# AIM-Harvard/pyradiomics

Hardware: NVIDIA H100
Metric: voxels/s full-texture voxel-based (higher is better)
Workload: dtype f64

## Files before the change

pyradiomics_b200/csrc/small_fast.cuh:

```cuda
#pragma once
#include "glcm_fast.cuh"

namespace rb {

struct SmallFastTables {
  double log2t[32];
  double inv2[256];
  double invsq[32];
  double rcp[64];
};

inline void small_fast_build_tables(SmallFastTables& T) {
  T.log2t[0] = 0; T.invsq[0] = 0; T.inv2[0] = 0; T.rcp[0] = 0;
  for (int c = 1; c < 32; c++) { T.log2t[c] = log2((double)c); T.invsq[c] = 1.0 / ((double)c * c); }
  for (int g = 1; g < 256; g++) T.inv2[g] = 1.0 / ((double)g * g);
  for (int c = 1; c < 64; c++) T.rcp[c] = 1.0 / (double)c;
}

RB_HD constexpr uint32_t nb26(int v) {
  uint32_t m = 0;
  const int z = v / 9, y = (v / 3) % 3, x = v % 3;
  for (int dz = -1; dz <= 1; dz++) for (int dy = -1; dy <= 1; dy++) for (int dx = -1; dx <= 1; dx++) {
    if (!dz && !dy && !dx) continue;
    const int z2 = z + dz, y2 = y + dy, x2 = x + dx;
    if (z2 < 0 || z2 > 2 || y2 < 0 || y2 > 2 || x2 < 0 || x2 > 2) continue;
    m |= 1u << (z2 * 9 + y2 * 3 + x2);
  }
  return m;
}
template <int V> struct NB26 { static constexpr uint32_t value = nb26(V); };

template <int V, int END> struct ForPos {
  template <typename F> static RB_HD void go(F& f) { f.template at<V>(); ForPos<V + 1, END>::go(f); }
};
template <int END> struct ForPos<END, END> { template <typename F> static RB_HD void go(F&) {} };

struct GldmPass1 {
  const int* wl; const uint32_t* cl; int* dep; uint32_t M;
  template <int V> RB_HD void at() { dep[V] = wl[V] ? (int)RB_POPC(cl[V] & NB26<V>::value) : -1 - V; }
};

RB_HD void gldm_fast_voxel(const int* wl, int alpha, const SmallFastTables& T, double* out) {
  uint32_t eq[27];
  RB_EQMASKS_27(wl, eq);
  uint32_t cl[27];
  if (alpha == 0) {
#pragma unroll
    for (int v = 0; v < 27; v++) cl[v] = eq[v];
  } else {
#pragma unroll
    for (int v = 0; v < 27; v++) cl[v] = 0;
#pragma unroll
    for (int p = 0; p < 27; p++)
#pragma unroll
      for (int q = p + 1; q < 27; q++) {
        const int d = wl[p] - wl[q];
        if (wl[p] && wl[q] && d <= alpha && -d <= alpha) { cl[p] |= 1u << q; cl[q] |= 1u << p; }
      }
  }
  int dep[27];
  GldmPass1 p1{wl, cl, dep, 0};
  ForPos<0, 27>::go(p1);
  uint32_t dq[27];
  RB_EQMASKS_27_KEY(dep, dq);
  int Nz = 0, Sj = 0, Sj2 = 0, B = 0, C = 0, X4 = 0, gl = 0, dn = 0;
  double Sinv = 0, A = 0, X1 = 0, X2 = 0, X3 = 0, lg = 0;
#pragma unroll
  for (int v = 0; v < 27; v++) {
    if (wl[v]) {
      const int g = wl[v], g2 = g * g, j = dep[v] + 1, j2 = j * j;
      const double ig = T.inv2[g], ij = T.invsq[j];
      Nz++; Sj += j; Sj2 += j2; B += g2; C += g; X4 += g2 * j2;
      Sinv += ij; A += ig; X1 += ig * ij; X2 += g2 * ij; X3 += j2 * ig;
      gl += RB_POPC(eq[v]); dn += RB_POPC(dq[v]);
      lg += T.log2t[RB_POPC(eq[v] & dq[v])];
    }
  }
  const double inv = 1.0 / Nz, inv2 = inv * inv;
  out[0] = T.log2t[Nz] - lg * inv;
  out[1] = dn * inv;
  out[2] = dn * inv2;
  out[3] = (double)(Nz * Sj2 - Sj * Sj) * inv2;
  out[4] = gl * inv;
  out[5] = (double)(Nz * B - C * C) * inv2;
  out[6] = B * inv;
  out[7] = Sj2 * inv;
  out[8] = X4 * inv;
  out[9] = X3 * inv;
  out[10] = A * inv;
  out[11] = Sinv * inv;
  out[12] = X2 * inv;
  out[13] = X1 * inv;
}

constexpr int NGTDM_L = 34034;

RB_HD constexpr int ngtdm_full_cnt(int v) {
  return (v % 3 == 1 ? 3 : 2) * ((v / 3) % 3 == 1 ? 3 : 2) * (v / 9 == 1 ? 3 : 2) - 1;
}

RB_HD double ngtdm_i2d(int d) {
#ifdef __CUDA_ARCH__
  return __hiloint2double(0x43300000, d) - 4503599627370496.0;
#else
  return (double)d;
#endif
}

RB_HD double ngtdm_complexity_pairs(const int* pk, const double* ns, int st, int nl, const SmallFastTables& T) {
  double c0 = 0, c1 = 0;
  for (int a = 0; a + 1 < nl; a++) {
    const int pa = pk[a * st], na = pa >> 8, ia = pa & 255;
    const double sa = ns[a * st];
    int b = a + 1;
    for (; b + 1 < nl; b += 2) {
      const int p0 = pk[b * st], p1 = pk[(b + 1) * st];
      const int x0 = ia - (p0 & 255), x1 = ia - (p1 & 255);
      c0 += ngtdm_i2d(x0 < 0 ? -x0 : x0) * ((sa + ns[b * st]) * T.rcp[na + (p0 >> 8)]);
      c1 += ngtdm_i2d(x1 < 0 ? -x1 : x1) * ((sa + ns[(b + 1) * st]) * T.rcp[na + (p1 >> 8)]);
    }
    if (b < nl) {
      const int p0 = pk[b * st], x0 = ia - (p0 & 255);
      c0 += ngtdm_i2d(x0 < 0 ? -x0 : x0) * ((sa + ns[b * st]) * T.rcp[na + (p0 >> 8)]);
    }
  }
  return c0 + c1;
}

struct NgtdmGeneralDiff {
  const int* wl; const uint32_t* eq; uint32_t M; const SmallFastTables* T; double* scr_ns; int st; double ssum;
  template <int V> RB_HD void at() {
    if (!wl[V]) return;
    constexpr uint32_t nb = NB26<V>::value;
    int sum = 0;
#pragma unroll
    for (int u = 0; u < 27; u++) if (nb >> u & 1u) sum += wl[u];
    const int cnt = RB_POPC(M & nb), x = cnt * wl[V] - sum;
    const double d = ngtdm_i2d(x < 0 ? -x : x) * T->rcp[cnt];
    ssum += d;
    const int r = RB_CTZ(eq[V]);
    const double prev = r == V ? 0.0 : scr_ns[r * st];
    scr_ns[r * st] = prev + d;
  }
};

template <bool FULL>
RB_HD void ngtdm_fast_body(const int* wl, const SmallFastTables& T, double* out, int* scr_pk, double* scr_ns, int st) {
  int B = 0, C = 0;
#pragma unroll
  for (int v = 0; v < 27; v++) { B += wl[v] * wl[v]; C += wl[v]; }
  uint32_t eq[27];
  RB_EQMASKS_27(wl, eq);
  int Nvp = 27, SE = 0;
  double ssum = 0;
  if (FULL) {
    int bx[27], by[27], bz[27];
#pragma unroll
    for (int r = 0; r < 27; r += 3) {
      bx[r] = wl[r] + wl[r + 1]; bx[r + 1] = bx[r] + wl[r + 2]; bx[r + 2] = wl[r + 1] + wl[r + 2];
    }
#pragma unroll
    for (int r = 0; r < 27; r += 9)
#pragma unroll
      for (int x = 0; x < 3; x++) {
        const int* b = bx + r + x;
        by[r + x] = b[0] + b[3]; by[r + 3 + x] = by[r + x] + b[6]; by[r + 6 + x] = b[3] + b[6];
      }
#pragma unroll
    for (int yx = 0; yx < 9; yx++) {
      bz[yx] = by[yx] + by[9 + yx]; bz[9 + yx] = bz[yx] + by[18 + yx]; bz[18 + yx] = by[9 + yx] + by[18 + yx];
    }
#pragma unroll
    for (int v = 0; v < 27; v++) {
      const int cnt = ngtdm_full_cnt(v);
      const int x = (cnt + 1) * wl[v] - bz[v];
      const int e = (x < 0 ? -x : x) * (NGTDM_L / cnt);
      SE += e;
      const int r = RB_CTZ(eq[v]);
      const int prev = r == v ? 0 : scr_pk[r * st];
      scr_pk[r * st] = prev + e;
    }
  } else {
    uint32_t M = 0;
#pragma unroll
    for (int v = 0; v < 27; v++) if (wl[v]) M |= 1u << v;
    Nvp = RB_POPC(M);
    NgtdmGeneralDiff p1{wl, eq, M, &T, scr_ns, st, 0.0};
    ForPos<0, 27>::go(p1);
    ssum = p1.ssum;
  }
  int nl = 0, SL = 0, SL2 = 0;
  double pw = 0;
  int X[27];
#pragma unroll
  for (int v = 0; v < 27; v++) {
    const bool rep = eq[v] && (eq[v] & ((1u << v) - 1)) == 0;
    const int n = RB_POPC(eq[v]), g = wl[v];
    const double ns = FULL ? ngtdm_i2d(n) * ngtdm_i2d(scr_pk[v * st]) : ngtdm_i2d(n) * scr_ns[v * st];
    scr_pk[nl * st] = n << 8 | g;
    scr_ns[nl * st] = ns;
    X[v] = rep ? g * n : 0;
    if (rep) { nl++; SL += g; SL2 += g * g; pw += ns; }
  }
  RB_NGTDM_SORT27(X);
  int bd = 0;
#pragma unroll
  for (int k = 0; k < 27; k++) bd += (2 * k - 53 + nl) * X[k];
  const double cpx = ngtdm_complexity_pairs(scr_pk, scr_ns, st, nl, T);
  const double u = FULL ? (double)NGTDM_L : 1.0, N = (double)Nvp;
  const double sdiff = FULL ? (double)SE : ssum;
  out[N_Coarseness] = pw != 0 ? N * u / pw : 1e6;
  const double div = (double)nl * (nl - 1);
  out[N_Contrast] = div != 0 ? 2.0 * (double)(Nvp * B - C * C) * sdiff / (N * N * N * u * div) : 0.0;
  out[N_Busyness] = bd != 0 ? pw / (2.0 * u * (double)bd) : 0.0;
  out[N_Complexity] = 2.0 * cpx / (N * u);
  out[N_Strength] = sdiff != 0 ? 2.0 * u * (double)(nl * B - 2 * C * SL + Nvp * SL2) / (N * sdiff) : 0.0;
}

RB_HD bool ngtdm_window_full(const int* wl) {
  bool full = true;
#pragma unroll
  for (int v = 0; v < 27; v++) full &= wl[v] != 0;
  return full;
}

RB_HD void ngtdm_fast_voxel(const int* wl, const SmallFastTables& T, double* out) {
  int pk[27] = {0};
  double ns[27] = {0};
  if (ngtdm_window_full(wl)) ngtdm_fast_body<true>(wl, T, out, pk, ns, 1);
  else ngtdm_fast_body<false>(wl, T, out, pk, ns, 1);
}

RB_HD uint32_t dilate26(uint32_t m) {
  constexpr uint32_t X0 = 0x1249249u, X2 = 0x4924924u;
  constexpr uint32_t Y0 = 0x01C0E07u, Y2 = 0x70381C0u;
  m |= ((m & ~X2) << 1) | ((m & ~X0) >> 1);
  m |= ((m & ~Y2) << 3) | ((m & ~Y0) >> 3);
  m |= (m << 9) | (m >> 9);
  return m & 0x7FFFFFFu;
}

struct GlszmAcc {
  int Nz, Sg, Sg2, Ss2, X4, gln;
  double A, Sinv, X1, X2, X3, lg;
  unsigned long long h0, h1, h2;
};

RB_HD void glszm_fast_voxel(const int* wl, const SmallFastTables& T, double* out) {
  uint32_t eq[27];
  RB_EQMASKS_27(wl, eq);
  uint32_t M = 0;
  uint32_t cls[13];
  int clg[13];
  int nl = 0, S_n = 0, S_g = 0, S_g2 = 0;
  double S_ig = 0;
#pragma unroll
  for (int v = 0; v < 27; v++) {
    if (wl[v]) M |= 1u << v;
    if (eq[v] && (eq[v] & ((1u << v) - 1)) == 0) {
      if (eq[v] == (1u << v)) { S_n++; S_g += wl[v]; S_g2 += wl[v] * wl[v]; S_ig += T.inv2[wl[v]]; }
      else { cls[nl] = eq[v]; clg[nl] = wl[v]; nl++; }
    }
  }
  GlszmAcc a;
  a.Nz = S_n; a.Sg = S_g; a.Sg2 = S_g2; a.Ss2 = S_n; a.X4 = S_g2; a.gln = S_n;
  a.A = S_ig; a.Sinv = (double)S_n; a.X1 = S_ig; a.X2 = (double)S_g2; a.X3 = S_ig; a.lg = 0;
  a.h0 = (unsigned long long)S_n; a.h1 = a.h2 = 0;
  for (int k = 0; k < nl; k++) {
    const int g = clg[k], g2 = g * g;
    uint32_t m = cls[k];
    const double ig = T.inv2[g];
    int zs[8];
    int zc = 0;
    while (m && zc < 8) {
      uint32_t comp = m & (0u - m);
      for (;;) {
        const uint32_t nx = dilate26(comp) & m;
        if (nx == comp) break;
        comp = nx;
      }
      m &= ~comp;
      const int sz = RB_POPC(comp), s2 = sz * sz;
      zs[zc++] = sz;
      const double is = T.invsq[sz];
      a.Nz++; a.Sg += g; a.Sg2 += g2; a.Ss2 += s2; a.X4 += g2 * s2;
      a.A += ig; a.Sinv += is; a.X1 += ig * is; a.X2 += g2 * is; a.X3 += s2 * ig;
      if (sz <= 12) a.h0 += 1ull << (5 * (sz - 1));
      else if (sz <= 24) a.h1 += 1ull << (5 * (sz - 13));
      else a.h2 += 1ull << (5 * (sz - 25));
    }
    a.gln += zc * zc;
    for (int k = 0; k < zc; k++) {
      int c = 0;
      for (int l = 0; l < zc; l++) c += zs[l] == zs[k];
      a.lg += T.log2t[c];
    }
  }
  int szn = 0;
#pragma unroll
  for (int k = 0; k < 12; k++) {
    const int c0 = (int)(a.h0 >> (5 * k)) & 31, c1 = (int)(a.h1 >> (5 * k)) & 31;
    szn += c0 * c0 + c1 * c1;
  }
#pragma unroll
  for (int k = 0; k < 3; k++) { const int c2 = (int)(a.h2 >> (5 * k)) & 31; szn += c2 * c2; }
  const int Np = RB_POPC(M), Nz = a.Nz;
  const double inv = 1.0 / Nz, inv2 = inv * inv;
  out[S_GLN] = a.gln * inv; out[S_GLNN] = a.gln * inv2;
  out[S_GLV] = (double)(Nz * a.Sg2 - a.Sg * a.Sg) * inv2;
  out[S_HGLE] = a.Sg2 * inv; out[S_LargeE] = a.Ss2 * inv; out[S_LargeHGLE] = a.X4 * inv; out[S_LargeLGLE] = a.X3 * inv;
  out[S_LGLE] = a.A * inv; out[S_SizeNU] = szn * inv; out[S_SizeNUN] = szn * inv2; out[S_SmallE] = a.Sinv * inv;
  out[S_SmallHGLE] = a.X2 * inv; out[S_SmallLGLE] = a.X1 * inv;
  out[S_Entropy] = T.log2t[Nz] - a.lg * inv;
  out[S_Percentage] = (double)Nz / Np;
  out[S_SizeVar] = (double)(Nz * a.Ss2 - Np * Np) * inv2;
}

}
```

pyradiomics_b200/csrc/voxel_fast.cu:

```cuda
#include <map>
#include <mutex>

#include "common.cuh"
#define RB_GLCM_BLOCK_SYNC 1
#include "glcm_fast.cuh"
#include "glcm_kernels.cuh"
#include "glrlm_fast.cuh"
#include "small_fast.cuh"
#include "host_common.hpp"

namespace rb {

bool glcm_fast_applicable(int cls, int level_bytes, const VoxParams& P) {
  return cls == C_GLCM && level_bytes == 1 && P.rz == 1 && P.ry == 1 && P.rx == 1 && P.na == 13 && P.symmetric &&
         !P.weighted && P.Ng <= 255;
}

struct GlcmQueue { GlcmTask* q = nullptr; double* res = nullptr; unsigned* count = nullptr; size_t cap = 0; };
static std::mutex g_queue_mu;
static std::map<std::pair<int, cudaStream_t>, GlcmQueue> g_queue_cache;
int glcm_release_queues() {
  int dev = 0;
  if (cudaGetDevice(&dev) != cudaSuccess) return RB_ERR_CUDA;
  cudaDeviceSynchronize();
  std::lock_guard<std::mutex> lk(g_queue_mu);
  for (auto it = g_queue_cache.begin(); it != g_queue_cache.end();) {
    if (it->first.first == dev) {
      cudaFree(it->second.q); cudaFree(it->second.res); cudaFree(it->second.count);
      it = g_queue_cache.erase(it);
    } else ++it;
  }
  return RB_OK;
}
static GlcmQueue* glcm_queue(cudaStream_t st, size_t need) {
  std::mutex& mu = g_queue_mu;
  auto& cache = g_queue_cache;
  int dev = 0;
  if (cudaGetDevice(&dev) != cudaSuccess) return nullptr;
  std::lock_guard<std::mutex> lk(mu);
  GlcmQueue& Q = cache[{dev, st}];
  if (!Q.count && cudaMalloc(&Q.count, sizeof(unsigned)) != cudaSuccess) return nullptr;
  if (Q.cap < need) {
    if (Q.q) { cudaStreamSynchronize(st); cudaFree(Q.q); cudaFree(Q.res); Q.q = nullptr; Q.res = nullptr; Q.cap = 0; }
    if (cudaMalloc(&Q.q, need * sizeof(GlcmTask)) != cudaSuccess) return nullptr;
    if (cudaMalloc(&Q.res, need * sizeof(double)) != cudaSuccess) { cudaFree(Q.q); Q.q = nullptr; return nullptr; }
    Q.cap = need;
  }
  return &Q;
}

int glcm_fast_launch(const void* lev, const uint8_t* centers, const VoxParams& P, double* out, long long fstride,
                     int z0, int z1, int out_z0, cudaStream_t st) {
  const GlcmFastTables* T = device_table<GlcmFastTables>([&](GlcmFastTables& h) { glcm_fast_build_tables(h, P.Ng); }, P.Ng);
  if (!T) return fail(RB_ERR_CUDA, "could not build the GLCM table block on the device");
  const long long plane = (long long)P.Y * P.X;
  if ((long long)(z1 - z0) * plane <= 0) return RB_OK;
  if (P.sy != P.X || P.sz != plane) return fail(RB_ERR_ARG, "GLCM fast path expects a contiguous level volume");
  const int sms = sm_count();
  const long long max_entries = 48ll << 20;
  int zchunk = (int)(max_entries / (plane * GF_NA));
  if (zchunk < 1) zchunk = 1;
  if (zchunk > z1 - z0) zchunk = z1 - z0;
  GlcmQueue* Q = glcm_queue(st, (size_t)zchunk * plane * GF_NA);
  if (!Q) return fail(RB_ERR_NOMEM, "could not allocate the GLCM eigen-task queue");
  constexpr int NT = 512;
  const int smem = glcm_phaseA_smem_bytes(NT);
  RB_CUDA(set_max_dynamic_smem(glcm_fast_kernel<1, NT>, smem));
  RB_CUDA(set_max_dynamic_smem(glcm_fast_solve_kernel<2>, GF_LZ_SMEM_BYTES));
  const uint8_t* l8 = (const uint8_t*)lev;
  for (int za = z0; za < z1; za += zchunk) {
    const int zb = za + zchunk < z1 ? za + zchunk : z1;
    RB_CUDA(cudaMemsetAsync(Q->count, 0, sizeof(unsigned), st));
    int grid = 0;
    RB_CUDA(resident_grid(glcm_fast_kernel<1, NT>, NT, smem, (long long)(zb - za) * plane, grid));
    glcm_fast_kernel<1, NT><<<grid, NT, smem, st>>>(l8, centers, P, T, out, fstride, za, zb, out_z0, Q->q, Q->count);
    RB_LAUNCH_CHECK();
    glcm_fast_solve_kernel<0><<<sms * 8, 128, 0, st>>>(l8, P, T, Q->q, Q->count, Q->res, 0);
    for (int g = 10; g <= 12; g += 2) glcm_fast_solve_kernel<1><<<sms * 8, 128, 0, st>>>(l8, P, T, Q->q, Q->count, Q->res, g);
    for (int g = 18; g >= 14; g -= 2)
      glcm_fast_solve_kernel<2><<<sms * 2, 128, GF_LZ_SMEM_BYTES, st>>>(l8, P, T, Q->q, Q->count, Q->res, g);
    RB_LAUNCH_CHECK();
    glcm_fast_finish_kernel<<<sms * 8, 256, 0, st>>>(P, Q->q, Q->count, Q->res, out + (long long)G_MCC * fstride, out_z0);
    RB_LAUNCH_CHECK();
  }
  return RB_OK;
}

__global__ void __launch_bounds__(128)
glrlm_fast_kernel(const uint8_t* __restrict__ lev, const uint8_t* __restrict__ centers,
                  const __grid_constant__ VoxParams P, const GlrlmFastTables* __restrict__ Tg,
                  double* __restrict__ out, long long fstride, int z0, int z1, int out_z0) {
  __shared__ GlrlmFastTables T;
  copy_tables_to_shared(T, Tg);
  __syncthreads();
  const long long plane = (long long)P.Y * P.X;
  const long long total = (long long)(z1 - z0) * plane;
  for (long long t = (long long)blockIdx.x * blockDim.x + threadIdx.x; t < total; t += (long long)gridDim.x * blockDim.x) {
    const ChunkVoxel v = chunk_voxel(P, plane, z0, out_z0, t);
    if (!chunk_center(lev, centers, plane, v)) {
#pragma unroll
      for (int k = 0; k < GLRLM_NF; k++) out[k * fstride + v.oi] = P.init_value;
      continue;
    }
    int wl[27];
    load_window27(lev, P, v.z, v.y, v.x, v.vi, true, wl, 1);
    double f[GLRLM_NF];
    glrlm_fast_voxel(wl, T, f);
#pragma unroll
    for (int k = 0; k < GLRLM_NF; k++) out[k * fstride + v.oi] = f[k];
  }
}

bool glrlm_fast_applicable(int cls, int level_bytes, const VoxParams& P) {
  return cls == C_GLRLM && level_bytes == 1 && P.rz == 1 && P.ry == 1 && P.rx == 1 && P.na == 13 && !P.weighted && P.Ng <= 255;
}

int glrlm_fast_launch(const void* lev, const uint8_t* centers, const VoxParams& P, double* out, long long fstride,
                      int z0, int z1, int out_z0, cudaStream_t st) {
  const GlrlmFastTables* T = device_table<GlrlmFastTables>(glrlm_fast_build_tables);
  if (!T) return fail(RB_ERR_CUDA, "could not build the GLRLM table block on the device");
  const long long total = (long long)(z1 - z0) * P.Y * P.X;
  if (total <= 0) return RB_OK;
  glrlm_fast_kernel<<<grid_for(total, 128, 32), 128, 0, st>>>((const uint8_t*)lev, centers, P, T, out, fstride, z0, z1, out_z0);
  RB_LAUNCH_CHECK();
  return RB_OK;
}

template <int CLS, int NT, bool SYNC>
__global__ void __launch_bounds__(NT)
small_fast_kernel(const uint8_t* __restrict__ lev, const uint8_t* __restrict__ centers,
                  const __grid_constant__ VoxParams P, const SmallFastTables* __restrict__ Tg,
                  double* __restrict__ out, long long fstride, int z0, int z1, int out_z0) {
  __shared__ SmallFastTables T;
  copy_tables_to_shared<NT>(T, Tg);
  __syncthreads();
  constexpr int NF = CLS == C_GLSZM ? GLSZM_NF : GLDM_NF;
  const long long plane = (long long)P.Y * P.X;
  const long long total = (long long)(z1 - z0) * plane;
  const long long ntiles = (total + NT - 1) / NT;
  for (long long tile = blockIdx.x; tile < ntiles; tile += gridDim.x) {
    if (SYNC) __syncthreads();
    const long long t = tile * NT + threadIdx.x;
    const bool live = t < total;
    if (!SYNC && !live) continue;
    const ChunkVoxel v = chunk_voxel(P, plane, z0, out_z0, t, live);
    const bool is_center = live && chunk_center(lev, centers, plane, v);
    if (!SYNC && !is_center) {
#pragma unroll
      for (int k = 0; k < NF; k++) out[k * fstride + v.oi] = P.init_value;
      continue;
    }
    int wl[27];
    load_window27(lev, P, v.z, v.y, v.x, v.vi, is_center, wl, 1);
    double f[16];
    if (CLS == C_GLSZM) glszm_fast_voxel(wl, T, f);
    else gldm_fast_voxel(wl, P.alpha, T, f);
    if (!live) continue;
#pragma unroll
    for (int k = 0; k < NF; k++) out[k * fstride + v.oi] = is_center ? f[k] : P.init_value;
  }
}

constexpr int NGTDM_NT = 128;
template <int NT>
__global__ void __launch_bounds__(NT, 4)
ngtdm_fast_kernel(const uint8_t* __restrict__ lev, const uint8_t* __restrict__ centers,
                  const __grid_constant__ VoxParams P, const SmallFastTables* __restrict__ Tg,
                  double* __restrict__ out, long long fstride, int z0, int z1, int out_z0) {
  __shared__ SmallFastTables T;
  __shared__ double ng_ns[27 * NT];
  __shared__ int ng_pk[27 * NT];
  __shared__ long long defer[2 * NT];
  __shared__ unsigned ndefer;
  copy_tables_to_shared<NT>(T, Tg);
  const int tid = threadIdx.x;
  if (tid == 0) ndefer = 0;
  __syncthreads();
  const long long plane = (long long)P.Y * P.X;
  full_window_tiles<NT>((long long)(z1 - z0) * plane, defer, ndefer,
    [&](long long t, bool live, auto defer_it) {
      if (!live) return;
      const ChunkVoxel v = chunk_voxel(P, plane, z0, out_z0, t);
      const bool is_center = chunk_center(lev, centers, plane, v);
      int wl[27];
      load_window27(lev, P, v.z, v.y, v.x, v.vi, is_center, wl, 1);
      if (is_center && ngtdm_window_full(wl)) {
        double f[NGTDM_NF];
        ngtdm_fast_body<true>(wl, T, f, ng_pk + tid, ng_ns + tid, NT);
#pragma unroll
        for (int k = 0; k < NGTDM_NF; k++) out[k * fstride + v.oi] = f[k];
      } else if (is_center) {
        defer_it();
      } else {
#pragma unroll
        for (int k = 0; k < NGTDM_NF; k++) out[k * fstride + v.oi] = P.init_value;
      }
    },
    [&](auto entry, bool live) {
      if (!live) return;
      const ChunkVoxel v = chunk_voxel(P, plane, z0, out_z0, entry());
      const bool is_center = chunk_center(lev, centers, plane, v);
      int wl[27];
      load_window27(lev, P, v.z, v.y, v.x, v.vi, is_center, wl, 1);
      double f[NGTDM_NF];
      ngtdm_fast_body<false>(wl, T, f, ng_pk + tid, ng_ns + tid, NT);
#pragma unroll
      for (int k = 0; k < NGTDM_NF; k++) out[k * fstride + v.oi] = f[k];
    });
}

bool small_fast_applicable(int cls, int level_bytes, const VoxParams& P) {
  return (cls == C_GLSZM || cls == C_GLDM || cls == C_NGTDM) && level_bytes == 1 && P.rz == 1 && P.ry == 1 && P.rx == 1 &&
         P.na == 26 && P.Ng <= 255;
}

int small_fast_launch(int cls, const void* lev, const uint8_t* centers, const VoxParams& P, double* out, long long fstride,
                      int z0, int z1, int out_z0, cudaStream_t st) {
  const SmallFastTables* T = device_table<SmallFastTables>(small_fast_build_tables);
  if (!T) return fail(RB_ERR_CUDA, "could not build the table block on the device");
  const long long total = (long long)(z1 - z0) * P.Y * P.X;
  if (total <= 0) return RB_OK;
  const uint8_t* l8 = (const uint8_t*)lev;
  if (cls == C_NGTDM) {
    int grid = 0;
    RB_CUDA(resident_grid(ngtdm_fast_kernel<NGTDM_NT>, NGTDM_NT, 0, total, grid));
    ngtdm_fast_kernel<NGTDM_NT><<<grid, NGTDM_NT, 0, st>>>(l8, centers, P, T, out, fstride, z0, z1, out_z0);
  } else if (cls == C_GLSZM) {
    small_fast_kernel<C_GLSZM, 128, false><<<grid_for(total, 128, 32), 128, 0, st>>>(l8, centers, P, T, out, fstride, z0, z1, out_z0);
  } else {
    small_fast_kernel<C_GLDM, 256, true><<<grid_for(total, 256, 16), 256, 0, st>>>(l8, centers, P, T, out, fstride, z0, z1, out_z0);
  }
  RB_LAUNCH_CHECK();
  return RB_OK;
}

}
```

Before: 263.9 million.

## Split GLSZM/GLDM voxel kernels into full-window fast path with deferred partial windows

Templates the GLSZM and GLDM per-voxel bodies on whether the 3x3x3 window is fully inside the mask, so the common case skips the zero checks and mask bookkeeping. Partial windows are deferred and handled in a second pass, reusing the NGTDM tiling scheme with a resident grid. GLDM computes its dependence histogram and joint entropy via packed counters and a combined key instead of a second equality-mask pass. GLSZM computes entropy incrementally with a delta-log table and keeps cluster scratch in shared memory, which adds shared memory use and relies on load_window27 returning a fullness flag.

```diff
diff --git a/pyradiomics_b200/csrc/small_fast.cuh b/pyradiomics_b200/csrc/small_fast.cuh
--- a/pyradiomics_b200/csrc/small_fast.cuh
+++ b/pyradiomics_b200/csrc/small_fast.cuh
@@ -8,6 +8,7 @@
   double inv2[256];
   double invsq[32];
   double rcp[64];
+  double dclog2[32];
 };
 
 inline void small_fast_build_tables(SmallFastTables& T) {
@@ -15,6 +16,7 @@
   for (int c = 1; c < 32; c++) { T.log2t[c] = log2((double)c); T.invsq[c] = 1.0 / ((double)c * c); }
   for (int g = 1; g < 256; g++) T.inv2[g] = 1.0 / ((double)g * g);
   for (int c = 1; c < 64; c++) T.rcp[c] = 1.0 / (double)c;
+  for (int c = 0; c < 32; c++) T.dclog2[c] = (c + 1) * log2((double)(c + 1)) - (c ? c * log2((double)c) : 0.0);
 }
 
 RB_HD constexpr uint32_t nb26(int v) {
@@ -36,13 +38,18 @@
 template <int END> struct ForPos<END, END> { template <typename F> static RB_HD void go(F&) {} };
 
 struct GldmPass1 {
-  const int* wl; const uint32_t* cl; int* dep; uint32_t M;
-  template <int V> RB_HD void at() { dep[V] = wl[V] ? (int)RB_POPC(cl[V] & NB26<V>::value) : -1 - V; }
-};
-
-RB_HD void gldm_fast_voxel(const int* wl, int alpha, const SmallFastTables& T, double* out) {
+  const uint32_t* cl; int* dep;
+  template <int V> RB_HD void at() { dep[V] = (int)RB_POPC(cl[V] & NB26<V>::value); }
+};
+
+template <bool FULL>
+RB_HD void gldm_fast_body(const int* wl, int alpha, const SmallFastTables& T, double* out) {
   uint32_t eq[27];
-  RB_EQMASKS_27(wl, eq);
+  if (FULL) RB_EQMASKS_27_KEY(wl, eq);
+  else RB_EQMASKS_27(wl, eq);
+  int gl = 0;
+#pragma unroll
+  for (int v = 0; v < 27; v++) gl += RB_POPC(eq[v]);
   uint32_t cl[27];
   if (alpha == 0) {
 #pragma unroll
@@ -55,28 +62,43 @@
 #pragma unroll
       for (int q = p + 1; q < 27; q++) {
         const int d = wl[p] - wl[q];
-        if (wl[p] && wl[q] && d <= alpha && -d <= alpha) { cl[p] |= 1u << q; cl[q] |= 1u << p; }
+        if ((FULL || (wl[p] && wl[q])) && d <= alpha && -d <= alpha) { cl[p] |= 1u << q; cl[q] |= 1u << p; }
       }
   }
   int dep[27];
-  GldmPass1 p1{wl, cl, dep, 0};
+  GldmPass1 p1{cl, dep};
   ForPos<0, 27>::go(p1);
-  uint32_t dq[27];
-  RB_EQMASKS_27_KEY(dep, dq);
-  int Nz = 0, Sj = 0, Sj2 = 0, B = 0, C = 0, X4 = 0, gl = 0, dn = 0;
+  int Nz = 0, Sj = 0, Sj2 = 0, B = 0, C = 0, X4 = 0;
   double Sinv = 0, A = 0, X1 = 0, X2 = 0, X3 = 0, lg = 0;
+  unsigned long long h0 = 0, h1 = 0, h2 = 0;
+  int key[27];
 #pragma unroll
   for (int v = 0; v < 27; v++) {
-    if (wl[v]) {
-      const int g = wl[v], g2 = g * g, j = dep[v] + 1, j2 = j * j;
+    const bool in = FULL || wl[v];
+    const int g = wl[v], g2 = g * g, j = dep[v] + 1, j2 = j * j;
+    key[v] = in ? g << 5 | dep[v] : -1 - v;
+    if (in) {
       const double ig = T.inv2[g], ij = T.invsq[j];
       Nz++; Sj += j; Sj2 += j2; B += g2; C += g; X4 += g2 * j2;
       Sinv += ij; A += ig; X1 += ig * ij; X2 += g2 * ij; X3 += j2 * ig;
-      gl += RB_POPC(eq[v]); dn += RB_POPC(dq[v]);
-      lg += T.log2t[RB_POPC(eq[v] & dq[v])];
-    }
-  }
-  const double inv = 1.0 / Nz, inv2 = inv * inv;
+      if (dep[v] < 12) h0 += 1ull << (5 * dep[v]);
+      else if (dep[v] < 24) h1 += 1ull << (5 * (dep[v] - 12));
+      else h2 += 1ull << (5 * (dep[v] - 24));
+    }
+  }
+  int dn = 0;
+#pragma unroll
+  for (int k = 0; k < 12; k++) { const int c = (int)(h0 >> (5 * k)) & 31; dn += c * c; }
+#pragma unroll
+  for (int k = 0; k < 12; k++) { const int c = (int)(h1 >> (5 * k)) & 31; dn += c * c; }
+#pragma unroll
+  for (int k = 0; k < 3; k++) { const int c = (int)(h2 >> (5 * k)) & 31; dn += c * c; }
+  uint32_t kq[27];
+  RB_EQMASKS_27_KEY(key, kq);
+#pragma unroll
+  for (int v = 0; v < 27; v++)
+    if (FULL || key[v] >= 0) lg += T.log2t[RB_POPC(kq[v])];
+  const double inv = FULL ? 1.0 / 27 : 1.0 / Nz, inv2 = inv * inv;
   out[0] = T.log2t[Nz] - lg * inv;
   out[1] = dn * inv;
   out[2] = dn * inv2;
@@ -217,7 +239,7 @@
   out[N_Strength] = sdiff != 0 ? 2.0 * u * (double)(nl * B - 2 * C * SL + Nvp * SL2) / (N * sdiff) : 0.0;
 }
 
-RB_HD bool ngtdm_window_full(const int* wl) {
+RB_HD bool window27_full(const int* wl) {
   bool full = true;
 #pragma unroll
   for (int v = 0; v < 27; v++) full &= wl[v] != 0;
@@ -227,7 +249,7 @@
 RB_HD void ngtdm_fast_voxel(const int* wl, const SmallFastTables& T, double* out) {
   int pk[27] = {0};
   double ns[27] = {0};
-  if (ngtdm_window_full(wl)) ngtdm_fast_body<true>(wl, T, out, pk, ns, 1);
+  if (window27_full(wl)) ngtdm_fast_body<true>(wl, T, out, pk, ns, 1);
   else ngtdm_fast_body<false>(wl, T, out, pk, ns, 1);
 }
 
@@ -246,20 +268,20 @@
   unsigned long long h0, h1, h2;
 };
 
-RB_HD void glszm_fast_voxel(const int* wl, const SmallFastTables& T, double* out) {
+template <bool FULL>
+RB_HD void glszm_fast_body(const int* wl, const SmallFastTables& T, double* out, unsigned long long* scr, int st) {
   uint32_t eq[27];
-  RB_EQMASKS_27(wl, eq);
+  if (FULL) RB_EQMASKS_27_KEY(wl, eq);
+  else RB_EQMASKS_27(wl, eq);
   uint32_t M = 0;
-  uint32_t cls[13];
-  int clg[13];
   int nl = 0, S_n = 0, S_g = 0, S_g2 = 0;
   double S_ig = 0;
 #pragma unroll
   for (int v = 0; v < 27; v++) {
-    if (wl[v]) M |= 1u << v;
+    if (!FULL && wl[v]) M |= 1u << v;
     if (eq[v] && (eq[v] & ((1u << v) - 1)) == 0) {
       if (eq[v] == (1u << v)) { S_n++; S_g += wl[v]; S_g2 += wl[v] * wl[v]; S_ig += T.inv2[wl[v]]; }
-      else { cls[nl] = eq[v]; clg[nl] = wl[v]; nl++; }
+      else { scr[nl * st] = eq[v] | (unsigned long long)wl[v] << 32; nl++; }
     }
   }
   GlszmAcc a;
@@ -267,12 +289,13 @@
   a.A = S_ig; a.Sinv = (double)S_n; a.X1 = S_ig; a.X2 = (double)S_g2; a.X3 = S_ig; a.lg = 0;
   a.h0 = (unsigned long long)S_n; a.h1 = a.h2 = 0;
   for (int k = 0; k < nl; k++) {
-    const int g = clg[k], g2 = g * g;
-    uint32_t m = cls[k];
+    const unsigned long long e = scr[k * st];
+    uint32_t m = (uint32_t)e;
+    const int g = (int)(e >> 32), g2 = g * g;
     const double ig = T.inv2[g];
-    int zs[8];
+    const unsigned long long l0 = a.h0, l1 = a.h1, l2 = a.h2;
     int zc = 0;
-    while (m && zc < 8) {
+    while (m) {
       uint32_t comp = m & (0u - m);
       for (;;) {
         const uint32_t nx = dilate26(comp) & m;
@@ -281,20 +304,17 @@
       }
       m &= ~comp;
       const int sz = RB_POPC(comp), s2 = sz * sz;
-      zs[zc++] = sz;
+      zc++;
       const double is = T.invsq[sz];
       a.Nz++; a.Sg += g; a.Sg2 += g2; a.Ss2 += s2; a.X4 += g2 * s2;
       a.A += ig; a.Sinv += is; a.X1 += ig * is; a.X2 += g2 * is; a.X3 += s2 * ig;
-      if (sz <= 12) a.h0 += 1ull << (5 * (sz - 1));
-      else if (sz <= 24) a.h1 += 1ull << (5 * (sz - 13));
-      else a.h2 += 1ull << (5 * (sz - 25));
+      int c;
+      if (sz <= 12) { c = (int)((a.h0 - l0) >> (5 * (sz - 1))) & 31; a.h0 += 1ull << (5 * (sz - 1)); }
+      else if (sz <= 24) { c = (int)((a.h1 - l1) >> (5 * (sz - 13))) & 31; a.h1 += 1ull << (5 * (sz - 13)); }
+      else { c = (int)((a.h2 - l2) >> (5 * (sz - 25))) & 31; a.h2 += 1ull << (5 * (sz - 25)); }
+      a.lg += T.dclog2[c];
     }
     a.gln += zc * zc;
-    for (int k = 0; k < zc; k++) {
-      int c = 0;
-      for (int l = 0; l < zc; l++) c += zs[l] == zs[k];
-      a.lg += T.log2t[c];
-    }
   }
   int szn = 0;
 #pragma unroll
@@ -304,16 +324,26 @@
   }
 #pragma unroll
   for (int k = 0; k < 3; k++) { const int c2 = (int)(a.h2 >> (5 * k)) & 31; szn += c2 * c2; }
-  const int Np = RB_POPC(M), Nz = a.Nz;
-  const double inv = 1.0 / Nz, inv2 = inv * inv;
+  const int Np = FULL ? 27 : RB_POPC(M), Nz = a.Nz;
+  const double inv = FULL ? T.rcp[Nz] : 1.0 / Nz, inv2 = inv * inv;
   out[S_GLN] = a.gln * inv; out[S_GLNN] = a.gln * inv2;
   out[S_GLV] = (double)(Nz * a.Sg2 - a.Sg * a.Sg) * inv2;
   out[S_HGLE] = a.Sg2 * inv; out[S_LargeE] = a.Ss2 * inv; out[S_LargeHGLE] = a.X4 * inv; out[S_LargeLGLE] = a.X3 * inv;
   out[S_LGLE] = a.A * inv; out[S_SizeNU] = szn * inv; out[S_SizeNUN] = szn * inv2; out[S_SmallE] = a.Sinv * inv;
   out[S_SmallHGLE] = a.X2 * inv; out[S_SmallLGLE] = a.X1 * inv;
   out[S_Entropy] = T.log2t[Nz] - a.lg * inv;
-  out[S_Percentage] = (double)Nz / Np;
+  out[S_Percentage] = FULL ? Nz * (1.0 / 27) : (double)Nz / Np;
   out[S_SizeVar] = (double)(Nz * a.Ss2 - Np * Np) * inv2;
 }
 
-}
+RB_HD void glszm_fast_voxel(const int* wl, const SmallFastTables& T, double* out) {
+  unsigned long long scr[13];
+  if (window27_full(wl)) glszm_fast_body<true>(wl, T, out, scr, 1);
+  else glszm_fast_body<false>(wl, T, out, scr, 1);
+}
+RB_HD void gldm_fast_voxel(const int* wl, int alpha, const SmallFastTables& T, double* out) {
+  if (window27_full(wl)) gldm_fast_body<true>(wl, alpha, T, out);
+  else gldm_fast_body<false>(wl, alpha, T, out);
+}
+
+}
diff --git a/pyradiomics_b200/csrc/voxel_fast.cu b/pyradiomics_b200/csrc/voxel_fast.cu
--- a/pyradiomics_b200/csrc/voxel_fast.cu
+++ b/pyradiomics_b200/csrc/voxel_fast.cu
@@ -126,39 +126,73 @@
   return RB_OK;
 }
 
-template <int CLS, int NT, bool SYNC>
-__global__ void __launch_bounds__(NT)
-small_fast_kernel(const uint8_t* __restrict__ lev, const uint8_t* __restrict__ centers,
-                  const __grid_constant__ VoxParams P, const SmallFastTables* __restrict__ Tg,
-                  double* __restrict__ out, long long fstride, int z0, int z1, int out_z0) {
+template <int CLS> struct TileClass;
+template <> struct TileClass<C_GLSZM> { static constexpr int NF = GLSZM_NF, NMG = 13; };
+template <> struct TileClass<C_GLDM> { static constexpr int NF = GLDM_NF, NMG = 0; };
+
+template <int CLS, bool FULL>
+__device__ __forceinline__ void tile_body(const int* wl, const SmallFastTables& T, int alpha, unsigned long long* mg,
+                                          int st, double* f) {
+  if constexpr (CLS == C_GLSZM) glszm_fast_body<FULL>(wl, T, f, mg, st);
+  else gldm_fast_body<FULL>(wl, alpha, T, f);
+}
+
+template <int CLS, int NT, int MINB>
+__global__ void __launch_bounds__(NT, MINB)
+tiles_fast_kernel(const uint8_t* __restrict__ lev, const uint8_t* __restrict__ centers, const __grid_constant__ VoxParams P,
+                  const SmallFastTables* __restrict__ Tg, double* __restrict__ out, long long fstride,
+                  int z0, int z1, int out_z0) {
+  using K = TileClass<CLS>;
   __shared__ SmallFastTables T;
+  __shared__ unsigned long long scr_mg[K::NMG * NT + 1];
+  __shared__ long long defer[2 * NT];
+  __shared__ unsigned ndefer;
   copy_tables_to_shared<NT>(T, Tg);
+  const int tid = threadIdx.x;
+  if (tid == 0) ndefer = 0;
   __syncthreads();
-  constexpr int NF = CLS == C_GLSZM ? GLSZM_NF : GLDM_NF;
-  const long long plane = (long long)P.Y * P.X;
-  const long long total = (long long)(z1 - z0) * plane;
-  const long long ntiles = (total + NT - 1) / NT;
-  for (long long tile = blockIdx.x; tile < ntiles; tile += gridDim.x) {
-    if (SYNC) __syncthreads();
-    const long long t = tile * NT + threadIdx.x;
-    const bool live = t < total;
-    if (!SYNC && !live) continue;
-    const ChunkVoxel v = chunk_voxel(P, plane, z0, out_z0, t, live);
-    const bool is_center = live && chunk_center(lev, centers, plane, v);
-    if (!SYNC && !is_center) {
-#pragma unroll
-      for (int k = 0; k < NF; k++) out[k * fstride + v.oi] = P.init_value;
-      continue;
-    }
-    int wl[27];
-    load_window27(lev, P, v.z, v.y, v.x, v.vi, is_center, wl, 1);
-    double f[16];
-    if (CLS == C_GLSZM) glszm_fast_voxel(wl, T, f);
-    else gldm_fast_voxel(wl, P.alpha, T, f);
-    if (!live) continue;
-#pragma unroll
-    for (int k = 0; k < NF; k++) out[k * fstride + v.oi] = is_center ? f[k] : P.init_value;
-  }
+  const long long plane = (long long)P.Y * P.X;
+  full_window_tiles<NT>((long long)(z1 - z0) * plane, defer, ndefer,
+    [&](long long t, bool live, auto defer_it) {
+      if (!live) return;
+      const ChunkVoxel v = chunk_voxel(P, plane, z0, out_z0, t);
+      const bool is_center = chunk_center(lev, centers, plane, v);
+      int wl[27];
+      const bool full = load_window27(lev, P, v.z, v.y, v.x, v.vi, is_center, wl, 1);
+      if (full) {
+        double f[K::NF];
+        tile_body<CLS, true>(wl, T, P.alpha, scr_mg + tid, NT, f);
+#pragma unroll
+        for (int k = 0; k < K::NF; k++) out[k * fstride + v.oi] = f[k];
+      } else if (is_center) {
+        defer_it();
+      } else {
+#pragma unroll
+        for (int k = 0; k < K::NF; k++) out[k * fstride + v.oi] = P.init_value;
+      }
+    },
+    [&](auto entry, bool live) {
+      if (!live) return;
+      const ChunkVoxel v = chunk_voxel(P, plane, z0, out_z0, entry());
+      int wl[27];
+      load_window27(lev, P, v.z, v.y, v.x, v.vi, true, wl, 1);
+      double f[K::NF];
+      tile_body<CLS, false>(wl, T, P.alpha, scr_mg + tid, NT, f);
+#pragma unroll
+      for (int k = 0; k < K::NF; k++) out[k * fstride + v.oi] = f[k];
+    });
+}
+
+constexpr int GLSZM_NT = 128, GLSZM_MINB = 4, GLDM_NT = 256, GLDM_MINB = 2;
+
+template <int CLS, int NT, int MINB>
+static int tiles_fast_launch(const SmallFastTables* T, const uint8_t* lev, const uint8_t* centers, const VoxParams& P,
+                             double* out, long long fstride, int z0, int z1, int out_z0, cudaStream_t st) {
+  int grid = 0;
+  RB_CUDA(resident_grid(tiles_fast_kernel<CLS, NT, MINB>, NT, 0, (long long)(z1 - z0) * P.Y * P.X, grid));
+  tiles_fast_kernel<CLS, NT, MINB><<<grid, NT, 0, st>>>(lev, centers, P, T, out, fstride, z0, z1, out_z0);
+  RB_LAUNCH_CHECK();
+  return RB_OK;
 }
 
 constexpr int NGTDM_NT = 128;
@@ -184,7 +218,7 @@
       const bool is_center = chunk_center(lev, centers, plane, v);
       int wl[27];
       load_window27(lev, P, v.z, v.y, v.x, v.vi, is_center, wl, 1);
-      if (is_center && ngtdm_window_full(wl)) {
+      if (is_center && window27_full(wl)) {
         double f[NGTDM_NF];
         ngtdm_fast_body<true>(wl, T, f, ng_pk + tid, ng_ns + tid, NT);
 #pragma unroll
@@ -225,13 +259,11 @@
     int grid = 0;
     RB_CUDA(resident_grid(ngtdm_fast_kernel<NGTDM_NT>, NGTDM_NT, 0, total, grid));
     ngtdm_fast_kernel<NGTDM_NT><<<grid, NGTDM_NT, 0, st>>>(l8, centers, P, T, out, fstride, z0, z1, out_z0);
-  } else if (cls == C_GLSZM) {
-    small_fast_kernel<C_GLSZM, 128, false><<<grid_for(total, 128, 32), 128, 0, st>>>(l8, centers, P, T, out, fstride, z0, z1, out_z0);
-  } else {
-    small_fast_kernel<C_GLDM, 256, true><<<grid_for(total, 256, 16), 256, 0, st>>>(l8, centers, P, T, out, fstride, z0, z1, out_z0);
-  }
-  RB_LAUNCH_CHECK();
-  return RB_OK;
-}
-
-}
+    RB_LAUNCH_CHECK();
+    return RB_OK;
+  }
+  if (cls == C_GLSZM) return tiles_fast_launch<C_GLSZM, GLSZM_NT, GLSZM_MINB>(T, l8, centers, P, out, fstride, z0, z1, out_z0, st);
+  return tiles_fast_launch<C_GLDM, GLDM_NT, GLDM_MINB>(T, l8, centers, P, out, fstride, z0, z1, out_z0, st);
+}
+
+}
```

After: 277.9 million (median of 6 runs). +5.3%, better.
